# nv-tlabs/LION

Measured on NVIDIA H100. Metric: shapes/sec (1000-step DDPM, 2048 latent pts, B=32), higher is better.
Workload: dtype tf32 (fp32 storage/accumulate)

## Files before the change

### include/lion_b200.h

```cpp
#ifndef LION_B200_H
#define LION_B200_H
#include <stddef.h>
#ifdef __cplusplus
extern "C" {
#endif

typedef struct LionCtx LionCtx;
typedef struct LionModel LionModel;

int lion_version(void);
const char* lion_last_error(void);
int lion_ctx_create(int device, LionCtx** out);
int lion_ctx_destroy(LionCtx* ctx);
int lion_ctx_last_launches(LionCtx* ctx);
int lion_ctx_last_conv_group(LionCtx* ctx);
int lion_ctx_last_conv_stage_taps(LionCtx* ctx);
int lion_ctx_set_conv_whole_slabs(LionCtx* ctx, int on);
int lion_ctx_set_sparse_conv1_dense(LionCtx* ctx, int on);
unsigned lion_ctx_generation(LionCtx* ctx);
int lion_ctx_timeline(LionCtx* ctx, unsigned long long* t_ns, char* names, int max_entries);
size_t lion_ctx_arena_bytes(LionCtx* ctx);
size_t lion_workspace_bytes(LionCtx* ctx);

int lion_avg_voxelize(const float* features, const int* coords, float* out, int* ind, int* cnt,
                      int B, int C, int N, int r, void* stream);
int lion_trilinear_devoxelize(const float* grid, const float* coords, float* out, int* inds, float* wgts,
                              int B, int C, int N, int r, int is_training, void* stream);
int lion_furthest_point_sampling(const float* coords, int* idx, int B, int N, int M, void* stream);
int lion_gather(const float* features, const int* idx, float* out, int B, int C, int N, int M, void* stream);
int lion_ball_query(const float* centers, const float* points, int* out, int B, int N, int M, float radius, int K,
                    void* stream);
int lion_grouping(const float* features, const int* idx, float* out, int B, int C, int N, int M, int U, void* stream);
int lion_three_nn_interpolate(const float* points, const float* centers, const float* centers_features, float* out,
                              int* idx, float* wgt, int B, int C, int N, int M, void* stream);
int lion_voxel_coords(const float* coords, float* norm_coords, int* vox, int B, int N, int r, int normalize, float eps,
                      void* stream);

int lion_avg_voxelize_backward(const float* grad_y , const int* ind , const int* cnt ,
                               float* grad_x , int B, int C, int N, int r, void* stream);
int lion_trilinear_devoxelize_backward(const float* grad_y , const int* inds , const float* wgts ,
                                       float* grad_x , int B, int C, int N, int r, void* stream);
// ... 138 lines not shown
```

### lion_b200/_lib.py

```python
import ctypes as C
import os
import threading

import torch

_HERE = os.path.dirname(os.path.abspath(__file__))
LIB_PATH = os.path.join(_HERE, "csrc", "liblion_b200.so")


class LionError(RuntimeError):
    pass


_lib = None
_lock = threading.Lock()
c_f = C.c_void_p


def _proto(lib):
    i, f, d, sz, vp = C.c_int, C.c_float, C.c_double, C.c_size_t, C.c_void_p
    P = lambda *a: list(a)
    sig = {
        "lion_version": ([], i),
        "lion_last_error": ([], C.c_char_p),
        "lion_ctx_create": (P(i, C.POINTER(vp)), i),
        "lion_ctx_destroy": (P(vp), i),
        "lion_ctx_last_launches": (P(vp), i),
        "lion_ctx_last_conv_group": (P(vp), i),
        "lion_ctx_last_conv_stage_taps": (P(vp), i),
        "lion_ctx_set_conv_whole_slabs": (P(vp, i), i),
        "lion_ctx_set_sparse_conv1_dense": (P(vp, i), i),
        "lion_ctx_arena_bytes": (P(vp), sz),
        "lion_ctx_generation": (P(vp), C.c_uint),
        "lion_ctx_timeline": (P(vp, vp, vp, i), i),
        "lion_avg_voxelize": (P(vp, vp, vp, vp, vp, i, i, i, i, vp), i),
        "lion_trilinear_devoxelize": (P(vp, vp, vp, vp, vp, i, i, i, i, i, vp), i),
        "lion_furthest_point_sampling": (P(vp, vp, i, i, i, vp), i),
        "lion_gather": (P(vp, vp, vp, i, i, i, i, vp), i),
        "lion_ball_query": (P(vp, vp, vp, i, i, i, f, i, vp), i),
        "lion_grouping": (P(vp, vp, vp, i, i, i, i, i, vp), i),
        "lion_three_nn_interpolate": (P(vp, vp, vp, vp, vp, vp, i, i, i, i, vp), i),
        "lion_voxel_coords": (P(vp, vp, vp, i, i, i, i, f, vp), i),
        "lion_avg_voxelize_backward": (P(vp, vp, vp, vp, i, i, i, i, vp), i),
        "lion_trilinear_devoxelize_backward": (P(vp, vp, vp, vp, i, i, i, i, vp), i),
        "lion_grouping_backward": (P(vp, vp, vp, i, i, i, i, i, vp), i),
        "lion_three_nn_interpolate_backward": (P(vp, vp, vp, vp, i, i, i, i, vp), i),
        "lion_gather_backward": (P(vp, vp, vp, i, i, i, i, vp), i),
        "lion_model_create": (P(vp, i, C.POINTER(i), i, C.POINTER(vp), i, C.POINTER(vp)), i),
        "lion_model_destroy": (P(vp), i),
        "lion_model_refresh": (P(vp), i),
        "lion_unet_forward": (P(vp, vp, vp, vp, vp, vp, i, i, vp), i),
        "lion_unet_forward_flags": (P(vp, vp, vp, vp, vp, vp, i, i, i, vp), i),
        "lion_unet_cache_style": (P(vp, vp, vp, i, vp), i),
        "lion_style_encoder_forward": (P(vp, vp, vp, i, i, vp), i),
# ... 232 lines not shown
```

### lion_b200/csrc/common.cuh

```cuda
#pragma once
#include <cuda_runtime.h>
#include <cstdint>
#include <cstdio>
#include <cstdarg>
#include <cstring>
#include <string>
#include <vector>
#include <mutex>

namespace lion {

enum : int { LION_OK = 0, LION_ERR_CUDA = -1, LION_ERR_ARG = -2, LION_ERR_OOM = -3, LION_ERR_STATE = -4 };

void set_error(const char* fmt, ...);
const char* get_error();

#define LION_CHECK_CUDA(expr)                                                          \
  do {                                                                                 \
    cudaError_t _e = (expr);                                                           \
    if (_e != cudaSuccess) {                                                           \
      lion::set_error("%s:%d: %s -> %s", __FILE__, __LINE__, #expr, cudaGetErrorString(_e)); \
      return lion::LION_ERR_CUDA;                                                      \
    }                                                                                  \
  } while (0)
// ... 14 lines not shown

constexpr int LION_MAX_STAMPS = 256;
struct Ctx {
  int device = 0;
  int num_sms = 132;
  int l2_bytes = 50 << 20;
  cudaStream_t stream = nullptr;
  cudaStream_t aux = nullptr;
  char* base = nullptr;
  char* zgrid = nullptr;
  size_t zgrid_cap = 0, zgrid_need = 0;
  size_t cap = 0;
  size_t off = 0;
  size_t peak = 0;
  unsigned generation = 0;
  std::mutex* mu = nullptr;
  bool dry = false;
  int launches = 0;
  int conv_smem_cap = 0;
  int conv_group_blocks = 0;
  int conv_stage_taps = 0;
  bool conv_whole_slabs = false;
  bool sparse_conv1_dense = false;
  unsigned long long* d_stamps = nullptr;
  int n_stamps = 0;
  char stamp_names[LION_MAX_STAMPS][24];

  void reset() { off = 0; peak = 0; launches = 0; zgrid_need = 0; n_stamps = 0; }
  void* alloc(size_t bytes) {
    size_t a = (off + 255) & ~size_t(255);
    off = a + bytes;
    if (off > peak) peak = off;
    if (dry) return (void*)(uintptr_t)(0x1000 + a);
    return base + a;
  }
  template <typename T> T* alloc_n(size_t n) { return (T*)alloc(n * sizeof(T)); }
  size_t mark() const { return off; }
  void release(size_t m) { off = m; }
};

int ctx_reserve(Ctx* c, size_t bytes);

#define LION_LAUNCH_ON(ctx, stream, kernel, grid, block, smem, ...)                    \
  do {                                                                                 \
    if (!(ctx)->dry) {                                                                 \
      kernel<<<(grid), (block), (smem), (stream)>>>(__VA_ARGS__);                      \
// ... 92 lines not shown
```

### lion_b200/csrc/conv_tc.cu

```cuda
#include <algorithm>
#include <type_traits>
#include <cuda_fp16.h>

#include "common.cuh"
#include "model.cuh"
#include "wgmma.cuh"

namespace lion {
namespace tc {

using namespace sm90;

constexpr int CONSUMER_WARPS = 8;
constexpr int THREADS = 32 * CONSUMER_WARPS + 32;
__host__ __device__ constexpr int conv_threads(int BPW) { return BPW == 2 ? 32 * CONSUMER_WARPS + 128 : THREADS; }
constexpr int PRODUCER_REGS = 96, CONSUMER_REGS = 200;
constexpr int MAX_A_STAGES = 16;
constexpr int MAX_B_STAGES = 4;
constexpr int OCC_SMEM = 1024;
__host__ __device__ constexpr int tiles_per_item(int NT) { return NT <= 32 ? 4 : (NT <= 64 ? 2 : 1); }
constexpr int SMEM_BIAS = 128 * 4, SMEM_BARS = 64 * 8 + 128;
__host__ __device__ constexpr int smem_stat(int NT) { return CONSUMER_WARPS * 2 * NT * 4; }
__host__ __device__ constexpr int smem_pool(int NT, int TPG) { return TPG == 1 ? CONSUMER_WARPS * 2 * NT * 4 : 0; }
__host__ __device__ constexpr int smem_fixed(int NT, int TPG) {
// ... 1 lines not shown
}

struct Params {
  const float4* in; const float* w; const float* bias; float4* out; double* ssum; double* ssq;
  int Gin, Gout_store, cout_pad;
  int rows;
  int p_begin, p_end;
  int ntile;
  int ntg, tpg;
  int tg_off[3];
  int tap_off[9];
  int r, rp, nzb, npl, nblk, ib;
  int halo;
  int KG, nchunk;
  int NT;
  int G;
  int B;
  int a_stage_bytes, b_stage_bytes, stage_rows;
  int a_stages;
  int b_stages;
  int tps;
  const unsigned char* occ;
  int occ_stride;
  float* pool_mm;
  int sched;
};

__host__ __device__ __forceinline__ int block_row(int k, int rp, int nzb, int npl) {
  const int x = k / npl, rem = k - x * npl, yb = rem / nzb, zb = rem - yb * nzb;
  return ((x + 1) * rp + 1 + 8 * yb) * rp + 1 + 8 * zb;
}

template <int KG, int TPG, int NT, int NB = 1, typename OP = float>
__device__ __forceinline__ void issue_stage(float (*d)[NT / 2], const uint32_t* a_addr, uint32_t b_addr, uint32_t a_pitch,
                                            uint32_t a_sbo, const int* tap_off) {
  const uint64_t b0 = make_desc(b_addr, NT * 16, 128);
  uint64_t a0[NB];
#pragma unroll
  for (int k = 0; k < NB; ++k) a0[k] = make_desc(a_addr[k], a_pitch, a_sbo);
#pragma unroll
  for (int t = 0; t < TPG; ++t) {
    const uint64_t toff = (uint64_t)(int64_t)(TPG == 1 ? 0 : tap_off[t]);
#pragma unroll
    for (int ks = 0; ks < KG / 2; ++ks)
#pragma unroll
      for (int k = 0; k < NB; ++k) {
// ... 30 lines not shown
    nt = (int)(u / per_nt);
    v0 = u - (long long)nt * per_nt;
    long long run = per_nt - v0;
    if (u_end - u < run) run = u_end - u;
    const long long k2 = (run + G - 1) / G;
    ntile = (int)((run + k2 - 1) / k2);
    u += ntile;
    return true;
  }
};
__device__ __forceinline__ Items make_items(long long U, int ntile_total, int B, int G, int sched) {
  const long long u_begin = U * blockIdx.x / gridDim.x, u_end = U * (blockIdx.x + 1) / gridDim.x;
  Items it{u_begin, u_end, ntile_total, B, G, 0, 0, 0, 0, 0, 0, 0, 0, 0};
  if (sched) {
    const int grid = (int)gridDim.x, q = (int)(U / grid), n_p = (int)(U - (long long)q * grid);
    const int tmax = q + (n_p ? 1 : 0);
    it.mode = 1; it.u = 0; it.u_end = 0;
    it.m = (tmax + G - 1) / G; it.q = q; it.n_p = n_p; it.n_q = grid - n_p;
    it.i = (int)blockIdx.x; it.c_i = (int)(u_begin - (long long)q * blockIdx.x);
    it.big = (int)(u_end - u_begin) > q; it.k = 0;
  }
  return it;
}

__device__ __forceinline__ void halo_mask(int p_lo, int rp, bool& ok_lo, bool& ok_hi) {
  const int p_hi = p_lo + 8;
  const int z0 = p_lo % rp, y0 = (p_lo / rp) % rp, z1 = p_hi % rp, y1 = (p_hi / rp) % rp;
  ok_lo = ok_lo && z0 >= 1 && z0 <= rp - 2 && y0 >= 1 && y0 <= rp - 2;
  ok_hi = ok_hi && z1 >= 1 && z1 <= rp - 2 && y1 >= 1 && y1 <= rp - 2;
}
template <int NT>
__device__ __forceinline__ void stat_add(float* s_stat, int cw, int lane, int col, float x0, float x1, float x2, float x3) {
  const float s0 = red8<0>(x0 + x2), s1 = red8<0>(x1 + x3);
  const float q0 = red8<0>(fmaf(x0, x0, x2 * x2)), q1 = red8<0>(fmaf(x1, x1, x3 * x3));
  if (lane < 4) {
    float* st = s_stat + (cw * 2) * NT + col;
    st[0] += s0; st[1] += s1; st[NT] += q0; st[NT + 1] += q1;
  }
}
template <int NT>
__device__ __forceinline__ void stat_flush(const Params& P, float* s_stat, int et, int b, int n0) {
  asm volatile("bar.sync 1, 256;" ::: "memory");
  if (et < NT) {
    float s = 0.f, qq = 0.f;
#pragma unroll
    for (int w = 0; w < CONSUMER_WARPS; ++w) {
// ... 50 lines not shown
      regs_dec<PRODUCER_REGS>();
      if (warp > CONSUMER_WARPS) return;
    }
    uint32_t sa = 0, pa = 0, sb = 0, pb = 0;
    const uint32_t bytes = (uint32_t)P.stage_rows * 16u;
    const uint32_t sA_addr = smem_u32(sA), sB_addr = smem_u32(sB);
    Items items = items0;
    int nt, ntile;
    long long v0;
    int occ_shape = -1;
    const int slab_floats = P.tpg * KG * NT * 4;
    auto copy_weights = [&](const float* src) {
      mbar_wait<SETREG>(bar_empty_b + 8 * sb, pb ^ 1);
      if (lane == 0) {
        mbar_expect_tx(bar_full_b + 8 * sb, P.b_stage_bytes);
        bulk_g2s(sB_addr + sb * (uint32_t)P.b_stage_bytes, src, P.b_stage_bytes, bar_full_b + 8 * sb);
      }
      if (++sb == B_STAGES) { sb = 0; pb ^= 1; }
    };
    while (items.next(nt, v0, ntile)) {
      const float* wsrc = P.w + (size_t)nt * P.nchunk * P.ntg * slab_floats;
      int my_b = 0, my_t = 0;
      if (lane < ntile) { const int vl = (int)v0 + lane; my_b = vl / ntile_total; my_t = vl - my_b * ntile_total; }
      for (int cc = 0; cc < P.nchunk; ++cc) {
        const int kg_real = min(KG, P.Gin - cc * KG);
        const size_t grp_lane = (size_t)(cc * KG + (lane < kg_real ? lane : 0));
        for (int tg = 0; tg < P.ntg; ++tg) {
          const bool may_skip = P.occ && !(cc == P.nchunk - 1 && tg == P.ntg - 1);
          const float* slab = wsrc + (size_t)(cc * P.ntg + tg) * slab_floats;
          copy_weights(slab);
          for (int j = 0; j < ntile; ++j) {
            const int bj = __shfl_sync(0xffffffffu, my_b, j), tj = __shfl_sync(0xffffffffu, my_t, j);
            long long row0;
            uint32_t cnt = (uint32_t)P.stage_rows;
            if (!BLK) {
              row0 = (long long)P.p_begin + (long long)tj * 128 - P.halo + P.tg_off[tg];
            } else {
              row0 = (long long)block_row(tj * P.ib, P.rp, P.nzb, P.npl) - P.rp - 1 + P.tg_off[tg];
              if (row0 + cnt > (long long)P.rows) cnt = (uint32_t)(P.rows - row0);
            }
            const float4* in_lane = P.in + ((size_t)bj * P.Gin + grp_lane) * P.rows;
            mbar_wait<SETREG>(bar_empty_a + 8 * sa, pa ^ 1);
            bool empty = false;
            if (may_skip) {
              const unsigned char* occ_b = P.occ + (size_t)bj * P.occ_stride;
              if (P.occ_stride <= OCC_SMEM) {
                if (occ_shape != bj) {
                  __syncwarp();
                  for (int k = lane; k < P.occ_stride; k += 32) s_occ[k] = __ldg(occ_b + k);
                  __syncwarp();
                  occ_shape = bj;
                }
                occ_b = s_occ;
              }
// ... 38 lines not shown
      if (s >= 0) { if (lane == 0) mbar_arrive(bar0 + 8 * s); s = -1; }
    };
    while (items.next(nt, v0, ntile)) {
#pragma unroll
      for (int j = 0; j < GT; ++j)
#pragma unroll
        for (int i = 0; i < NACC; ++i) acc[j][i] = 0.0f;
      int g_f = 0, nbw = 0;
      uint32_t boff[GT];
      if (BLK) {
        const int g_b = (int)(v0 / ntile_total);
        g_f = (int)(v0 - (long long)g_b * ntile_total) * P.ib;
        const int nb = min(P.ib, P.nblk - g_f);
        nbw = (nb - wg + 1) / 2;
        const int s_f = block_row(g_f, P.rp, P.nzb, P.npl);
#pragma unroll
        for (int j = 0; j < GT; ++j) {
          const int k = 2 * j + wg < nb ? g_f + 2 * j + wg : g_f;
          boff[j] = (uint32_t)(block_row(k, P.rp, P.nzb, P.npl) - s_f + P.rp + 1) * 16u;
        }
      }
      int pend_a = -1, pend_b = -1;
      bool skip[BLK ? 1 : GT];
      for (int cc = 0; cc < P.nchunk; ++cc) {
        for (int tg = 0; tg < P.ntg; ++tg) {
          const uint32_t sa0 = sa, pa0 = pa;
#pragma unroll
          for (int s = 0; s < NPARTS; ++s) {
            mbar_wait<SETREG>(bar_full_b + 8 * sb, pb);
            const uint32_t b_addr = b_ring + sb * (uint32_t)P.b_stage_bytes;
            const int* toff = P.tap_off + s * TPS;
            bool issued = false;
            sa = sa0; pa = pa0;
#pragma unroll
            for (int j = 0; j < (BLK ? 1 : GT); ++j) {
              if (j < ntile) {
                if (s == 0) {
                  mbar_wait<SETREG>(bar_full_a + 8 * sa, pa);
                  skip[j] = s_skip[sa] != 0;
                  if (skip[j]) { int st = (int)sa; release(st, bar_empty_a); }
                }
                if (!skip[j]) {
                  const uint32_t a_addr = a_ring + sa * (uint32_t)P.a_stage_bytes;
                  wg_fence();
                  if (!BLK) {
                    issue_stage<KG, TPS, NT, 1, OP>(&acc[j], &a_addr, b_addr, a_pitch, a_sbo, toff);
                  } else {
                    uint32_t a_blk[GT];
#pragma unroll
                    for (int k = 0; k < GT; ++k) a_blk[k] = a_addr + boff[k];
                    issue_stage<KG, TPS, NT, GT, OP>(acc, a_blk, b_addr, a_pitch, a_sbo, toff);
                  }
                  wg_commit();
                  wg_wait<1>();
                  release(pend_a, bar_empty_a);
                  release(pend_b, bar_empty_b);
                  if (s == NPARTS - 1) pend_a = (int)sa;
                  issued = true;
                }
                if (++sa == (uint32_t)A_STAGES) { sa = 0; pa ^= 1; }
              }
            }
            if (pend_b >= 0) {
              wg_wait<0>();
              release(pend_a, bar_empty_a);
              release(pend_b, bar_empty_b);
            }
            if (issued) pend_b = (int)sb;
            else { int st = (int)sb; release(st, bar_empty_b); }
            if (++sb == B_STAGES) { sb = 0; pb ^= 1; }
          }
        }
      }
      wg_wait<0>();
      release(pend_a, bar_empty_a);
      release(pend_b, bar_empty_b);
#pragma unroll
      for (int j = 0; j < GT; ++j) fence_regs<NACC>(acc[j]);

      const int n0 = nt * NT;
      asm volatile("bar.sync 1, 256;" ::: "memory");
      if (et < NT) s_bias[et] = P.bias ? P.bias[n0 + et] : 0.0f;
      asm volatile("bar.sync 1, 256;" ::: "memory");
      int b = (int)(v0 / ntile_total);
#pragma unroll
      for (int j = 0; j < GT; ++j) {
        if (j < (BLK ? nbw : ntile)) {
          int tj = 0, p_lo, p_hi;
          bool ok_lo, ok_hi;
          bool in_lo, in_hi;
          if (!BLK) {
            const long long vj = v0 + j;
            const int bj = (int)(vj / ntile_total);
            tj = (int)(vj - (long long)bj * ntile_total);
            if (bj != b) { if (P.ssum) stat_flush<NT>(P, s_stat, et, b, n0); b = bj; }
            p_lo = P.p_begin + tj * 128 + r_lo; p_hi = p_lo + 8;
            in_lo = p_lo < P.p_end; in_hi = p_hi < P.p_end;
            ok_lo = in_lo; ok_hi = in_hi;
            if (TPG != 1) halo_mask(p_lo, P.rp, ok_lo, ok_hi);
          } else {
            const int k = g_f + 2 * j + wg, x = k / P.npl, rem = k - x * P.npl, yb = rem / P.nzb, zb = rem - yb * P.nzb;
            const int y = 1 + 8 * yb + 2 * wq, z = 1 + 8 * zb + (lane >> 2);
            p_lo = ((x + 1) * P.rp + y) * P.rp + z; p_hi = p_lo + P.rp;
            ok_lo = y <= P.r && z <= P.r; ok_hi = y + 1 <= P.r && z <= P.r;
            in_lo = ok_lo; in_hi = ok_hi;
          }
#pragma unroll
          for (int i = 0; i < NT / 8; ++i) {
            const int col = 8 * i + c_lo;
            const float x0 = ok_lo ? acc[j][4 * i + 0] + s_bias[col] : 0.0f, x1 = ok_lo ? acc[j][4 * i + 1] + s_bias[col + 1] : 0.0f;
            const float x2 = ok_hi ? acc[j][4 * i + 2] + s_bias[col] : 0.0f, x3 = ok_hi ? acc[j][4 * i + 3] + s_bias[col + 1] : 0.0f;
            if (P.ssum) stat_add<NT>(s_stat, cw, lane, col, x0, x1, x2, x3);
            if (TPG == 1 && P.pool_mm) {
              const float mn0 = red8<1>(fminf(x0, x2)), mn1 = red8<1>(fminf(x1, x3));
              const float mx0 = red8<2>(fmaxf(x0, x2)), mx1 = red8<2>(fmaxf(x1, x3));
              if (lane < 4) {
                float* sp = s_pool + (cw * 2) * NT + col;
                sp[0] = mn0; sp[1] = mn1; sp[NT] = mx0; sp[NT + 1] = mx1;
              }
            } else {
              const float y0 = __shfl_xor_sync(0xffffffffu, odd ? x0 : x2, 1);
              const float y1 = __shfl_xor_sync(0xffffffffu, odd ? x1 : x3, 1);
              const int g = (n0 + 8 * i + (lane & 2) * 2) >> 2;
              if (g < P.Gout_store) {
                float4* o = P.out + ((size_t)b * P.Gout_store + g) * P.rows;
                if (!odd && in_lo) o[p_lo] = make_float4(x0, x1, y0, y1);
                if (odd && in_hi) o[p_hi] = make_float4(y0, y1, x2, x3);
              }
            }
          }
          if (TPG == 1 && P.pool_mm) {
            const int bar_id = 2 + wg;
            asm volatile("bar.sync %0, 128;" ::"r"(bar_id) : "memory");
            const long long ncent = (long long)P.rows / 32;
            for (int e = et - 128 * wg; e < 2 * NT; e += 128) {
              const int k = e / NT, c = e - k * NT;
              const float* s0 = s_pool + ((4 * wg + 2 * k) * 2) * NT + c;
              const float* s1 = s0 + 2 * NT;
              const float mn = fminf(s0[0], s1[0]), mx = fmaxf(s0[NT], s1[NT]);
              const long long centre = (long long)(P.p_begin + tj * 128 + 64 * wg + 32 * k) >> 5;
              const int ch = n0 + c;
              float* dst = P.pool_mm + ((((size_t)b * (P.cout_pad / 4) + (ch >> 2)) * ncent + centre) * 2) * 4 + (ch & 3);
              dst[0] = mn; dst[4] = mx;
            }
            asm volatile("bar.sync %0, 128;" ::"r"(bar_id) : "memory");
          }
        }
      }
      if (P.ssum) stat_flush<NT>(P, s_stat, et, b, n0);
    }
// ... 113 lines not shown
  });
  return 0;
}

int conv_tc_prepare_f16(Model* m, ConvW& w) {
  if (w.tc16.w || !w.tc.w || w.ntaps != 27 || w.cin_pad != w.cout_pad || w.cout != w.cout_pad) return 0;
  if (!(w.cout_pad == 32 || w.cout_pad == 64 || w.cout_pad == 128)) return 0;
  ConvTcW t = w.tc;
  const int G = w.cin_pad / 8;
  t.KG = conv_tc_kg(w.ntaps, t.NT, G);
  t.nchunk = (G + t.KG - 1) / t.KG;
  if (!((t.NT == 32 && t.KG == 4) || (t.NT == 64 && t.KG == 8) || (t.NT == 128 && t.KG == 4))) return 0;
  const size_t total = (size_t)(w.cout_pad / t.NT) * t.nchunk * t.ntg * t.tpg * t.KG * t.NT * 8;
  __half* w16 = nullptr;
  LION_TRY(m->dmalloc(&w16, total));
  t.w = reinterpret_cast<float*>(w16);
  w.tc16 = t;
  m->repack.push_back([t, w16, wt = w.wt, ntaps = w.ntaps, cin_pad = w.cin_pad, cout_pad = w.cout_pad, total] {
    tc::k_pack_tc16<<<(unsigned)cdivz(total, 256), 256>>>(wt, w16, ntaps, cin_pad, cout_pad, t.NT, t.nchunk, t.ntg, t.tpg, t.KG);
  });
  return 0;
}

bool conv_tc_usable(const ConvW& w, const ConvGeom& geo) {
  if (!w.tc.w) return false;
  if (geo.ntaps != w.ntaps) return false;
  return true;
}

int conv_tc_run(Ctx* c, const ConvW& w, const float4* in, int Gin, float4* out, int Gout_store, double* ssum, double* ssq,
                const ConvGeom& geo, int B, float* pool_mm, bool f16) {
  tc::Params P{};
  if (f16 && !w.tc16.w) { set_error("conv_tc: no FP16 packing of this convolution"); return LION_ERR_STATE; }
  const ConvTcW& T = f16 ? w.tc16 : w.tc;
  if (pool_mm && (w.ntaps != 1 || geo.p_begin != 0 || geo.p_end != geo.rows || geo.rows % 128)) {
    set_error("conv_tc: the pooled epilogue needs a 1x1 convolution over a multiple of 128 rows"); return LION_ERR_ARG;
  }
  P.pool_mm = pool_mm;
  const int NT = T.NT, KG = T.KG, tpg = T.tpg;
  P.in = in; P.w = T.w; P.bias = w.bias; P.out = out; P.ssum = ssum; P.ssq = ssq;
  P.Gin = Gin; P.Gout_store = Gout_store; P.cout_pad = w.cout_pad;
  P.rows = geo.rows; P.p_begin = geo.p_begin; P.p_end = geo.p_end;
  P.ntg = T.ntg; P.tpg = tpg; P.KG = KG; P.nchunk = T.nchunk; P.NT = NT;
  const int slab_bytes = tpg * KG * NT * 16;
  P.B = B;
  P.occ = geo.occ; P.occ_stride = geo.occ_stride;
  const size_t fixed = tc::smem_fixed(NT, tpg);
  const bool blk = w.ntaps == 27 && NT == 128;
  const int ntile_rows = cdiv(geo.p_end - geo.p_begin, 128);
  int ntile;
  P.halo = 0;
  if (w.ntaps == 27) {
    const int rp = geo.rp, r = rp - 2;
    for (int dx = 0; dx < 3; ++dx) P.tg_off[dx] = (dx - 1) * rp * rp;
    for (int dy = 0; dy < 3; ++dy) for (int dz = 0; dz < 3; ++dz) P.tap_off[dy * 3 + dz] = (dy - 1) * rp + (dz - 1);
    P.r = r; P.rp = rp;
  } else {
    P.tg_off[0] = 0; P.tap_off[0] = 0;
  }
  const int n_tiles_n = w.cout_pad / NT;
  if (blk) {
    const int rp = P.rp, r = P.r;
    P.nzb = cdiv(r, 8); P.npl = P.nzb * P.nzb; P.nblk = r * P.npl;
    auto window_rows = [&](int ib) {
      int wrows = 0;
      for (int f = 0; f < P.nblk; f += ib) {
        const int l = std::min(f + ib, P.nblk) - 1;
        wrows = std::max(wrows, tc::block_row(l, rp, P.nzb, P.npl) - tc::block_row(f, rp, P.nzb, P.npl) + 9 * rp + 10);
      }
// ... 25 lines not shown
    }
    int a_stages = (int)((227LL * 1024 - (long long)fixed - b_stages * stage) / P.a_stage_bytes);
    if (c->conv_smem_cap > 0 && a_stages >= 5) {
      const int capped = (int)(((long long)c->conv_smem_cap - (long long)fixed - b_stages * stage) / P.a_stage_bytes);
      if (capped >= 4 && capped < a_stages) a_stages = capped;
    }
    a_stages = std::min(a_stages, tc::MAX_A_STAGES);
    return a_stages >= 2 ? a_stages : 0;
  };
  int b_whole = 0, b_parts = 0;
  const int a_whole = ring(tpg, b_whole);
  const int a_parts = blk && !c->conv_whole_slabs ? ring(3, b_parts) : 0;
  const bool parts = a_parts > a_whole && a_parts >= P.G + 1;
  if (!parts && !a_whole) {
    set_error("conv_tc: shared memory cannot hold the operand pipeline (N=%d, KG=%d)", NT, KG); return LION_ERR_ARG;
  }
  P.tps = parts ? 3 : tpg;
  P.b_stage_bytes = slab_bytes / tpg * P.tps;
  P.b_stages = parts ? b_parts : b_whole;
  const int a_stages = parts ? a_parts : a_whole;
  P.a_stages = a_stages;
  const int b_stages = P.b_stages;
  if (!blk && P.occ && a_stages < 2 * P.G) P.occ = nullptr;
  size_t smem = (size_t)a_stages * P.a_stage_bytes + (size_t)b_stages * P.b_stage_bytes + fixed;
  if (smem > 227 * 1024) { set_error("conv_tc: %zu bytes of shared memory needed", smem); return LION_ERR_ARG; }
  auto grid_for = [&](int nt_per_shape) {
    long long n_units = (long long)nt_per_shape * n_tiles_n * B;
    long long per_cta = (n_units + c->num_sms - 1) / c->num_sms;
    return (int)((n_units + per_cta - 1) / per_cta);
  };
  const int grid = grid_for(ntile);
  tc::Params S = P;
  if (blk && ssum) {
    P.ssum = nullptr; P.ssq = nullptr;
    S.ntile = ntile_rows; S.G = tc::tiles_per_item(NT);
  }
  auto stats = [&]() -> int {
    if (!(blk && ssum)) return 0;
    LION_LAUNCH(c, tc::k_conv_stats<128>, grid_for(ntile_rows), 256, 0, S);
    return check_launch(c, "conv_tc stats");
  };
  const int bpw = blk ? P.ib / 2 : 1;
  c->conv_group_blocks = blk ? P.ib : 0;
  c->conv_stage_taps = P.tps;
#define CONV_TC_CASE_OP(kg, tpg_, nt_, blk_, bpw_, tps_, op)                                              \
  if (f16 == std::is_same<op, __half>::value && KG == kg && tpg == tpg_ && NT == nt_ && blk == blk_ && bpw == bpw_ && P.tps == tps_) { \
// ... 27 lines not shown
```

### lion_b200/csrc/model.cuh

```cuda
#pragma once
#include <functional>
#include <memory>
#include <vector>
#include "common.cuh"

namespace lion {

struct StyleLayer { const float* w; const float* b; int n_out; int out_off; };

struct ConvTcW {
  float* w = nullptr;
  int NT = 0;
  int KG = 0;
  int nchunk = 0;
  int ntg = 0, tpg = 0;
};

struct Cursor {
  const float* const* p;
  int n, i = 0;
  bool bad = false;
  const float* next() {
    if (i >= n) { bad = true; return nullptr; }
    return p[i++];
// ... 131 lines not shown
  }
  ~Model() {
    for (void* q : owned) cudaFree(q);
    for (cudaEvent_t e : events) cudaEventDestroy(e);
    if (aff_cache) cudaFree(aff_cache);
    if (gp) global_prior_free(gp);
  }
};


int make_conv(Model* m, ConvW& w, const float* w_src, const float* b_src, int ntaps, int cin_ref, int cout,
              const std::vector<int>& kmap);
std::vector<int> ident_map(int c);
static inline int roundup(int a, int b) { return (a + b - 1) / b * b; }

struct ConvGeom {
  int ntaps;
  int off[27];
  int rp;
  int rows;
  int p_begin, p_end;
  const unsigned char* occ;
  int occ_stride;
};

int conv_tc_prepare(Model* m, ConvW& w);
int conv_tc_prepare_f16(Model* m, ConvW& w);
bool conv_tc_usable(const ConvW& w, const ConvGeom& geo);
bool ygemm_usable(const ConvW& y);
int ygemm_run(Ctx* c, const ConvW& y, const float4* xc, float* out, int ld, const int* nocc, int B, int N);
bool sa_fused_usable(const SABlk& s);
int sa_fused_run(Ctx* c, const SABlk& s, const float4* feat, const float4* points, const float4* centers, const int* nidx,
                 const float* scale1, const float* shift1, double* ssum, double* ssq, int stat_stride, float* pool_mm,
                 int B, int N);
int conv_tc_run(Ctx* c, const ConvW& w, const float4* in, int Gin, float4* out, int Gout_store, double* ssum,
                double* ssq, const ConvGeom& geo, int B, float* pool_mm = nullptr, bool f16 = false);

}
```

### lion_b200/csrc/net.cu

```cuda
#include <algorithm>
#include <deque>
#include <memory>
#include <cstdlib>
#include <cmath>
#include "common.cuh"
#include "packed_kernels.cuh"
#include "model.cuh"
#include "../../include/lion_b200.h"

namespace lion {

static thread_local char g_err[1024] = "";
void set_error(const char* fmt, ...) {
  va_list ap;
  va_start(ap, fmt);
  vsnprintf(g_err, sizeof(g_err), fmt, ap);
  va_end(ap);
}
const char* get_error() { return g_err; }

int ctx_reserve(Ctx* c, size_t bytes) {
  if (bytes <= c->cap) return 0;
  cudaStreamCaptureStatus st = cudaStreamCaptureStatusNone;
  cudaStreamIsCapturing(c->stream, &st);
// ... 519 lines not shown
      LION_CHECK_CUDA(cudaFuncSetAttribute(k_act_grid<false>, cudaFuncAttributePreferredSharedMemoryCarveout, cudaSharedmemCarveoutMaxShared));
      LION_CHECK_CUDA(cudaFuncSetAttribute(k_act_grid<true>, cudaFuncAttributePreferredSharedMemoryCarveout, cudaSharedmemCarveoutMaxShared));
      LION_CHECK_CUDA(cudaFuncSetAttribute(k_scatter_compact, cudaFuncAttributePreferredSharedMemoryCarveout, cudaSharedmemCarveoutMaxShared));
    }
    const dim3 grid(cdiv(r * r * r, 32 * nwarp), f.B);
    unsigned* mask = f.c->alloc_n<unsigned>((size_t)f.B * cdiv(r * r * r, 32));
    const bool whole = whole_raw || f.c->sparse_conv1_dense;
    if (p.c1.cout_pad == 32)
      LION_LAUNCH(f.c, k_sparse_conv_gather<32>, grid, 32 * nwarp, smem, y, ld, vp->vgrid, p.c1.bias, raw1, s1, q1, p.c1.cout_pad, r, N,
                  mask, whole);
    else
      LION_LAUNCH(f.c, k_sparse_conv_gather<64>, grid, 32 * nwarp, smem, y, ld, vp->vgrid, p.c1.bias, raw1, s1, q1, p.c1.cout_pad, r, N,
                  mask, whole);
    LION_TRY(check_launch(f.c, "sparse conv1"));
    o.ssum = s1; o.ssq = q1;
    o.mask = mask;
  } else {
    LION_TRY(alloc_stats(f, p.c1.cout_pad, &o.ssum, &o.ssq));
    LION_TRY(run_conv(f, p.c1, o.g_in, Gin, raw1, Gout, o.ssum, o.ssq, geo1));
  }
  return 0;
}

static int pvconv_fwd(Fwd& f, const PVConvBlk& p, PF feat, const float4* c4, float4* dst, int Gd, int g_off) {
  int N = feat.R, r = p.r, rp = r + 2, P = rp * rp * rp, Gin = p.cin / 4, Gout = p.cout / 4;
  if (feat.G != Gin) { set_error("PVConv: got %d input channels, expected %d", feat.G * 4, p.cin); return LION_ERR_ARG; }
  VoxPrep* vp;
  LION_TRY(get_vox(f, f.c->stream, c4, N, r, &vp));
  size_t mk = f.c->mark();
  ConvGeom geo = geom_grid(r);
  const ConvW& pw = p.point.conv[0];
  PF rawp;
  AffSrc ap;
  PrepJob jp, j1;
  Conv1Out c1;
  LION_TRY(pvconv_conv1(f, p, feat, vp, 0, f.pv != nullptr, c1, [&]() -> int {
    rawp = alloc_pf(f, Gout, N);
    return conv_gn_deferred(f, pw, feat.p, feat.G, rawp.p, Gout, geom_rows(N), p.point.gn[0], (double)N, ap, jp);
  }));
  const bool sparse1 = c1.sparse;
  float4 *raw1 = c1.raw, *g_in = c1.g_in;
  const unsigned* mask1 = f.c->sparse_conv1_dense ? nullptr : c1.mask;
  AffSrc a1;
  const double V = (double)r * r * r;
  j1 = prep_job(f, p.g1, c1.ssum, c1.ssq, p.c1.cout_pad, V, nullptr, nullptr, a1);
  LION_TRY(run_prep(f, j1, &jp));
  stamp(f.c, f.c->stream, " conv1");
  const bool h2 = f.conv_f16 && p.c2.tc16.w;
  const int Gact = h2 ? Gout / 2 : Gout;
  float4* act1 = alloc_vg(f, Gact, r);
  LION_TRY(poison_vg(f, act1, Gact, r));
  {
    const int nb_act = cdiv(P, 256 * ACT_U);
    const dim3 grid(nb_act + (sparse1 ? 0 : cdiv(N, 256)), Gact, f.B);
    if (h2)
      LION_LAUNCH(f.c, k_act_grid<true>, grid, 256, 0, raw1, act1, a1, Gout, p.cout, rp, P, nb_act, vp->ppos, g_in, Gin, N, mask1,
                  p.c1.bias);
    else
      LION_LAUNCH(f.c, k_act_grid<false>, grid, 256, 0, raw1, act1, a1, Gout, p.cout, rp, P, nb_act, vp->ppos, g_in, Gin, N, mask1,
                  p.c1.bias);
  }
  stamp(f.c, f.c->stream, " act1");
  float4* raw2 = alloc_vg(f, Gout, r);
  LION_TRY(poison_vg(f, raw2, Gout, r));
  AffSrc a2;
  LION_TRY(conv_gn(f, p.c2, act1, Gact, raw2, Gout, geo, p.g2, V, p.se1, p.se2, a2, h2));
  stamp(f.c, f.c->stream, " conv2");
  if (f.pv) {
    PvRecord& R = *f.pv;
    R.raw1 = raw1; R.act1 = act1; R.raw2 = raw2; R.rawp = rawp.p; R.act1_f16 = h2;
    R.a1 = a1; R.ap = ap; R.a2 = a2;
    R.conv2 = !conv_tc_usable(p.c2, geo) ? 0 : f.c->conv_group_blocks ? f.c->conv_group_blocks : 1;
  }
  if (p.has_attn) {
    PF fused = alloc_pf(f, Gout, N);
    LION_LAUNCH(f.c, k_devox_fuse, dim3(cdiv(N, 128), Gout, f.B), 128, 0, raw2, vp->nc, a2.scale, a2.shift, rawp.p, ap,
                fused.p, Gout, p.cout, N, r, P, Gout, 0);
    LION_TRY(check_launch(f.c, "pvconv"));
    if (f.pv) f.pv->fused = fused.p;
    if (Gd != Gout || g_off != 0) {
      PF t = alloc_pf(f, Gout, N);
      LION_TRY(attn_fwd(f, p.attn, fused, t.p, Gout, 0));
      LION_LAUNCH(f.c, k_copy_groups, dim3(cdiv(N, 256), Gout, f.B), 256, 0, t.p, dst, Gout, Gd, g_off, N);
    } else {
      LION_TRY(attn_fwd(f, p.attn, fused, dst, Gd, g_off));
    }
  } else {
    LION_LAUNCH(f.c, k_devox_fuse, dim3(cdiv(N, 128), Gout, f.B), 128, 0, raw2, vp->nc, a2.scale, a2.shift, rawp.p, ap,
                dst, Gout, p.cout, N, r, P, Gd, g_off);
// ... 500 lines not shown
}

}

using namespace lion;

struct LionCtx { Ctx c; std::mutex mu; };
struct LionModel { Model m; };

extern "C" int lion_version(void) { return 100; }
extern "C" const char* lion_last_error(void) { return get_error(); }

extern "C" int lion_ctx_create(int device, LionCtx** out) {
  LION_REQUIRE(out, "lion_ctx_create: null out");
  LION_CHECK_CUDA(cudaSetDevice(device));
  LionCtx* h = new LionCtx();
  h->c.device = device;
  h->c.mu = &h->mu;
  cudaDeviceProp prop;
  LION_CHECK_CUDA(cudaGetDeviceProperties(&prop, device));
  h->c.num_sms = prop.multiProcessorCount;
  h->c.l2_bytes = prop.l2CacheSize;
  LION_CHECK_CUDA(cudaStreamCreateWithFlags(&h->c.aux, cudaStreamNonBlocking));
  { const char* e = getenv("LION_TIMELINE");
    if (e && atoi(e) != 0) LION_CHECK_CUDA(cudaMalloc(&h->c.d_stamps, LION_MAX_STAMPS * sizeof(unsigned long long))); }
  if (prop.major != 9 || prop.minor != 0) {
    set_error("lion_b200 is built for sm_90a only; device %d is sm_%d%d", device, prop.major, prop.minor);
    delete h;
    return LION_ERR_STATE;
  }
  *out = h;
  return 0;
}
extern "C" int lion_ctx_destroy(LionCtx* h) {
  if (!h) return 0;
  if (h->c.base) cudaFree(h->c.base);
  if (h->c.zgrid) cudaFree(h->c.zgrid);
  if (h->c.aux) cudaStreamDestroy(h->c.aux);
  if (h->c.d_stamps) cudaFree(h->c.d_stamps);
  delete h;
  return 0;
}
extern "C" int lion_ctx_last_launches(LionCtx* h) { return h ? h->c.launches : 0; }
extern "C" int lion_ctx_last_conv_group(LionCtx* h) { return h ? h->c.conv_group_blocks : 0; }
extern "C" int lion_ctx_last_conv_stage_taps(LionCtx* h) { return h ? h->c.conv_stage_taps : 0; }
extern "C" int lion_ctx_set_conv_whole_slabs(LionCtx* h, int on) {
  LION_REQUIRE(h, "lion_ctx_set_conv_whole_slabs: null context");
  h->c.conv_whole_slabs = on != 0;
  return 0;
}
extern "C" int lion_ctx_set_sparse_conv1_dense(LionCtx* h, int on) {
  LION_REQUIRE(h, "lion_ctx_set_sparse_conv1_dense: null context");
  h->c.sparse_conv1_dense = on != 0;
  return 0;
}
extern "C" unsigned lion_ctx_generation(LionCtx* h) { return h ? h->c.generation : 0; }
extern "C" int lion_ctx_timeline(LionCtx* h, unsigned long long* t_ns, char* names, int max_entries) {
  LION_REQUIRE(h && t_ns && names && max_entries >= 0, "lion_ctx_timeline: null argument");
  if (!h->c.d_stamps) { set_error("lion_ctx_timeline: the context was created without LION_TIMELINE=1"); return LION_ERR_STATE; }
  int n = h->c.n_stamps < max_entries ? h->c.n_stamps : max_entries;
  LION_CHECK_CUDA(cudaSetDevice(h->c.device));
  LION_CHECK_CUDA(cudaDeviceSynchronize());
  LION_CHECK_CUDA(cudaMemcpy(t_ns, h->c.d_stamps, (size_t)n * sizeof(unsigned long long), cudaMemcpyDeviceToHost));
  for (int i = 0; i < n; ++i) memcpy(names + (size_t)i * 24, h->c.stamp_names[i], 24);
  return n;
}
extern "C" size_t lion_ctx_arena_bytes(LionCtx* h) { return h ? h->c.cap : 0; }
extern "C" size_t lion_workspace_bytes(LionCtx* h) { return h ? h->c.cap + h->c.zgrid_cap : 0; }

extern "C" int lion_model_create(LionCtx* ctx, int kind, const int* desc, int ndesc, const float* const* params,
                                 int nparams, LionModel** out) {
  LION_REQUIRE(ctx && out && (desc || ndesc == 0) && (params || nparams == 0), "lion_model_create: null argument");
  LION_CHECK_CUDA(cudaSetDevice(ctx->c.device));
  std::unique_ptr<LionModel> h(new LionModel());
  Model* m = &h->m;
  m->ctx = &ctx->c; m->kind = kind;
// ... 690 lines not shown
```

### lion_b200/csrc/packed_kernels.cuh

```cuda
#pragma once
#include <cuda_fp16.h>
#include "common.cuh"
#include "point_core.cuh"
#include "model.cuh"

namespace lion {

__device__ __forceinline__ float4 f4_max(float4 a, float4 b) {
  return make_float4(fmaxf(a.x, b.x), fmaxf(a.y, b.y), fmaxf(a.z, b.z), fmaxf(a.w, b.w));
}
__device__ __forceinline__ float4 f4_scale(float4 a, float s) { return make_float4(a.x * s, a.y * s, a.z * s, a.w * s); }
__device__ __forceinline__ float4 f4_add(float4 a, float4 b) { return make_float4(a.x + b.x, a.y + b.y, a.z + b.z, a.w + b.w); }
__device__ __forceinline__ float4 f4_fma(float4 a, float s, float4 c) {
  return make_float4(fmaf(a.x, s, c.x), fmaf(a.y, s, c.y), fmaf(a.z, s, c.z), fmaf(a.w, s, c.w));
}

__global__ void k_make_coords(const float4* __restrict__ x, float4* __restrict__ c4, int total) {
  int i = blockIdx.x * blockDim.x + threadIdx.x;
  if (i >= total) return;
  float4 v = x[i];
  v.w = 0.0f;
  c4[i] = v;
}

// ... 198 lines not shown
#pragma unroll
  for (int k = 0; k < CPL; ++k) { cs[0][k] = cs[1][k] = 0.0f; cq[0][k] = cq[1][k] = 0.0f; }
  const int nlive = max(0, min(32, V - word * 32));
  for (int j = 0; j < nlive; j += 2) {
#pragma unroll
    for (int h = 0; h < 2; ++h) {
      if (j + h < nlive) {
#pragma unroll
        for (int k = 0; k < CPL; ++k) { const float a = acc[(j + h) * PITCH + lane * CPL + k]; cs[h][k] += a; cq[h][k] = fmaf(a, a, cq[h][k]); }
      }
    }
  }
#pragma unroll
  for (int k = 0; k < CPL; ++k) { s_red[0][wid][lane * CPL + k] = cs[0][k] + cs[1][k]; s_red[1][wid][lane * CPL + k] = cq[0][k] + cq[1][k]; }
  __syncthreads();
  if (threadIdx.x < C) {
    float a = 0.0f, qq = 0.0f;
    for (int w = 0; w < nw; ++w) { a += s_red[0][w][threadIdx.x]; qq += s_red[1][w][threadIdx.x]; }
    atomicAdd(ssum + (size_t)b * stat_stride + threadIdx.x, (double)a);
    atomicAdd(ssq + (size_t)b * stat_stride + threadIdx.x, (double)qq);
  }
}

__global__ void k_scatter(const float4* __restrict__ feat, const int* __restrict__ s_order, const int* __restrict__ s_ppos,
                          const int* __restrict__ s_len, float4* __restrict__ grid, int G, int N, int P) {
  int b = blockIdx.z, g = blockIdx.y;
  int s = blockIdx.x * blockDim.x + threadIdx.x;
  if (s >= N) return;
  int pp = s_ppos[(size_t)b * N + s];
  if (pp < 0) return;
  int len = s_len[(size_t)b * N + s];
  float inv = 1.0f / (float)len;
  const float4* f = feat + ((size_t)b * G + g) * N;
  const int* ord = s_order + (size_t)b * N + s;
  float4 acc = f4_scale(f[ord[0]], inv);
  for (int k = 1; k < len; ++k) acc = f4_add(acc, f4_scale(f[ord[k]], inv));
  grid[((size_t)b * G + g) * P + pp] = acc;
}


template <int COT>
__global__ void __launch_bounds__(128)
k_conv_simt(const float4* __restrict__ in, const float* __restrict__ Wt, const float* __restrict__ bias,
            float4* __restrict__ out, double* __restrict__ ssum, double* __restrict__ ssq,
            int Gin, int cin_pad, int cout_pad, int Gout_store, ConvGeom geo) {
  extern __shared__ float s_w[];
// ... 745 lines not shown
```

Measured before the change: 3.214.

## Skip conv2 tiles whose 3x3x3 neighbourhood has no occupied voxels, using class-valued outputs

For the second PVConv convolution, a flag kernel marks 64-voxel blocks whose whole 3x3x3 neighbourhood holds no occupied conv1 voxels. For such blocks the input is just the activated bias, so the output depends only on boundary class. A tiny 5x5x5 class grid is convolved once, and the tensor-core conv skips the MMA for flagged tiles and copies the class values instead. This adds a flag kernel, a small extra conv and branching in the producer/consumer pipeline, which could stall the pipeline when tiles are only partly live.

```diff
diff --git a/include/lion_b200.h b/include/lion_b200.h
--- a/include/lion_b200.h
+++ b/include/lion_b200.h
@@ -17,6 +17,8 @@
 int lion_ctx_last_conv_stage_taps(LionCtx* ctx);
 int lion_ctx_set_conv_whole_slabs(LionCtx* ctx, int on);
 int lion_ctx_set_sparse_conv1_dense(LionCtx* ctx, int on);
+int lion_ctx_set_conv2_class_mode(LionCtx* ctx, int mode);
+int lion_ctx_last_conv2_class_blocks(LionCtx* ctx, long long* flagged, long long* total);
 unsigned lion_ctx_generation(LionCtx* ctx);
 int lion_ctx_timeline(LionCtx* ctx, unsigned long long* t_ns, char* names, int max_entries);
 size_t lion_ctx_arena_bytes(LionCtx* ctx);
diff --git a/lion_b200/_lib.py b/lion_b200/_lib.py
--- a/lion_b200/_lib.py
+++ b/lion_b200/_lib.py
@@ -30,6 +30,8 @@
         "lion_ctx_last_conv_stage_taps": (P(vp), i),
         "lion_ctx_set_conv_whole_slabs": (P(vp, i), i),
         "lion_ctx_set_sparse_conv1_dense": (P(vp, i), i),
+        "lion_ctx_set_conv2_class_mode": (P(vp, i), i),
+        "lion_ctx_last_conv2_class_blocks": (P(vp, vp, vp), i),
         "lion_ctx_arena_bytes": (P(vp), sz),
         "lion_ctx_generation": (P(vp), C.c_uint),
         "lion_ctx_timeline": (P(vp, vp, vp, i), i),
diff --git a/lion_b200/csrc/common.cuh b/lion_b200/csrc/common.cuh
--- a/lion_b200/csrc/common.cuh
+++ b/lion_b200/csrc/common.cuh
@@ -60,6 +60,9 @@
   int conv_stage_taps = 0;
   bool conv_whole_slabs = false;
   bool sparse_conv1_dense = false;
+  int conv2_class_mode = 0;
+  unsigned long long* d_cls_count = nullptr;
+  long long cls_blocks = 0;
   unsigned long long* d_stamps = nullptr;
   int n_stamps = 0;
   char stamp_names[LION_MAX_STAMPS][24];
diff --git a/lion_b200/csrc/conv_tc.cu b/lion_b200/csrc/conv_tc.cu
--- a/lion_b200/csrc/conv_tc.cu
+++ b/lion_b200/csrc/conv_tc.cu
@@ -47,6 +47,10 @@
   int tps;
   const unsigned char* occ;
   int occ_stride;
+  const unsigned char* cls_flag;
+  int cls_stride;
+  const float4* cls;
+  int cls_store;
   float* pool_mm;
   int sched;
 };
@@ -123,6 +127,8 @@
   }
   return it;
 }
+
+__device__ __forceinline__ int cls_of(int v, int r) { return v <= 1 ? 0 : (v >= r ? 2 : 1); }
 
 __device__ __forceinline__ void halo_mask(int p_lo, int rp, bool& ok_lo, bool& ok_hi) {
   const int p_hi = p_lo + 8;
@@ -219,6 +225,12 @@
       const float* wsrc = P.w + (size_t)nt * P.nchunk * P.ntg * slab_floats;
       int my_b = 0, my_t = 0;
       if (lane < ntile) { const int vl = (int)v0 + lane; my_b = vl / ntile_total; my_t = vl - my_b * ntile_total; }
+      unsigned live = (1u << ntile) - 1u;
+      if (!BLK && P.cls_flag) {
+        const unsigned char* fl = P.cls_flag + (size_t)my_b * P.cls_stride + 2 * my_t;
+        live = __ballot_sync(0xffffffffu, lane < ntile && !(__ldg(fl) && __ldg(fl + 1)));
+      }
+      if (!live) continue;
       for (int cc = 0; cc < P.nchunk; ++cc) {
         const int kg_real = min(KG, P.Gin - cc * KG);
         const size_t grp_lane = (size_t)(cc * KG + (lane < kg_real ? lane : 0));
@@ -227,6 +239,7 @@
           const float* slab = wsrc + (size_t)(cc * P.ntg + tg) * slab_floats;
           copy_weights(slab);
           for (int j = 0; j < ntile; ++j) {
+            if (!((live >> j) & 1u)) continue;
             const int bj = __shfl_sync(0xffffffffu, my_b, j), tj = __shfl_sync(0xffffffffu, my_t, j);
             long long row0;
             uint32_t cnt = (uint32_t)P.stage_rows;
@@ -311,7 +324,22 @@
       }
       int pend_a = -1, pend_b = -1;
       bool skip[BLK ? 1 : GT];
-      for (int cc = 0; cc < P.nchunk; ++cc) {
+      unsigned live = (1u << ntile) - 1u, mine = ~0u;
+      if (!BLK && P.cls_flag) {
+        live = 0u; mine = 0u;
+#pragma unroll
+        for (int j = 0; j < GT; ++j) {
+          if (j < ntile) {
+            const long long vj = v0 + j;
+            const int bj = (int)(vj / ntile_total), tj = (int)(vj - (long long)bj * ntile_total);
+            const unsigned char* fl = P.cls_flag + (size_t)bj * P.cls_stride + 2 * tj;
+            const bool f0 = __ldg(fl) != 0, f1 = __ldg(fl + 1) != 0;
+            if (!(f0 && f1)) live |= 1u << j;
+            if (!(wg ? f1 : f0)) mine |= 1u << j;
+          }
+        }
+      }
+      for (int cc = 0; cc < (live ? P.nchunk : 0); ++cc) {
         for (int tg = 0; tg < P.ntg; ++tg) {
           const uint32_t sa0 = sa, pa0 = pa;
 #pragma unroll
@@ -323,10 +351,10 @@
             sa = sa0; pa = pa0;
 #pragma unroll
             for (int j = 0; j < (BLK ? 1 : GT); ++j) {
-              if (j < ntile) {
+              if ((live >> j) & 1u) {
                 if (s == 0) {
                   mbar_wait<SETREG>(bar_full_a + 8 * sa, pa);
-                  skip[j] = s_skip[sa] != 0;
+                  skip[j] = s_skip[sa] != 0 || !((mine >> j) & 1u);
                   if (skip[j]) { int st = (int)sa; release(st, bar_empty_a); }
                 }
                 if (!skip[j]) {
@@ -357,6 +385,11 @@
             }
             if (issued) pend_b = (int)sb;
             else { int st = (int)sb; release(st, bar_empty_b); }
+            if ((live & ~mine) && pend_b >= 0) {
+              wg_wait<0>();
+              release(pend_a, bar_empty_a);
+              release(pend_b, bar_empty_b);
+            }
             if (++sb == B_STAGES) { sb = 0; pb ^= 1; }
           }
         }
@@ -387,6 +420,20 @@
             in_lo = p_lo < P.p_end; in_hi = p_hi < P.p_end;
             ok_lo = in_lo; ok_hi = in_hi;
             if (TPG != 1) halo_mask(p_lo, P.rp, ok_lo, ok_hi);
+            if (!((mine >> j) & 1u)) {
+              const float4* cb = P.cls + (size_t)b * (P.cout_pad / 4) * 125 + n0 / 4;
+#pragma unroll
+              for (int h = 0; h < 2; ++h) {
+                const int p = h ? p_hi : p_lo, x = p / (P.rp * P.rp), y = (p / P.rp) % P.rp, z = p % P.rp;
+                const int row = ((cls_of(x, P.r) + 1) * 5 + cls_of(y, P.r) + 1) * 5 + cls_of(z, P.r) + 1;
+                const float* src = reinterpret_cast<const float*>(cb + ((lane & 3) >> 1) * 125 + row) + 2 * (lane & 1);
+#pragma unroll
+                for (int i = 0; i < NT / 8; ++i) {
+                  const float2 v = __ldg(reinterpret_cast<const float2*>(src + (size_t)2 * 125 * 4 * i));
+                  acc[j][4 * i + 2 * h] = v.x; acc[j][4 * i + 2 * h + 1] = v.y;
+                }
+              }
+            }
           } else {
             const int k = g_f + 2 * j + wg, x = k / P.npl, rem = k - x * P.npl, yb = rem / P.nzb, zb = rem - yb * P.nzb;
             const int y = 1 + 8 * yb + 2 * wq, z = 1 + 8 * zb + (lane >> 2);
@@ -394,11 +441,13 @@
             ok_lo = y <= P.r && z <= P.r; ok_hi = y + 1 <= P.r && z <= P.r;
             in_lo = ok_lo; in_hi = ok_hi;
           }
+          const bool cmp = (mine >> j) & 1u, st = cmp || P.cls_store;
 #pragma unroll
           for (int i = 0; i < NT / 8; ++i) {
             const int col = 8 * i + c_lo;
-            const float x0 = ok_lo ? acc[j][4 * i + 0] + s_bias[col] : 0.0f, x1 = ok_lo ? acc[j][4 * i + 1] + s_bias[col + 1] : 0.0f;
-            const float x2 = ok_hi ? acc[j][4 * i + 2] + s_bias[col] : 0.0f, x3 = ok_hi ? acc[j][4 * i + 3] + s_bias[col + 1] : 0.0f;
+            float x0 = acc[j][4 * i + 0], x1 = acc[j][4 * i + 1], x2 = acc[j][4 * i + 2], x3 = acc[j][4 * i + 3];
+            if (cmp) { x0 += s_bias[col]; x1 += s_bias[col + 1]; x2 += s_bias[col]; x3 += s_bias[col + 1]; }
+            x0 = ok_lo ? x0 : 0.0f; x1 = ok_lo ? x1 : 0.0f; x2 = ok_hi ? x2 : 0.0f; x3 = ok_hi ? x3 : 0.0f;
             if (P.ssum) stat_add<NT>(s_stat, cw, lane, col, x0, x1, x2, x3);
             if (TPG == 1 && P.pool_mm) {
               const float mn0 = red8<1>(fminf(x0, x2)), mn1 = red8<1>(fminf(x1, x3));
@@ -413,8 +462,8 @@
               const int g = (n0 + 8 * i + (lane & 2) * 2) >> 2;
               if (g < P.Gout_store) {
                 float4* o = P.out + ((size_t)b * P.Gout_store + g) * P.rows;
-                if (!odd && in_lo) o[p_lo] = make_float4(x0, x1, y0, y1);
-                if (odd && in_hi) o[p_hi] = make_float4(y0, y1, x2, x3);
+                if (!odd && in_lo && st) o[p_lo] = make_float4(x0, x1, y0, y1);
+                if (odd && in_hi && st) o[p_hi] = make_float4(y0, y1, x2, x3);
               }
             }
           }
@@ -574,6 +623,8 @@
   return 0;
 }
 
+bool conv_tc_row_tiles_3x3(const ConvW& w) { return w.tc.w && w.ntaps == 27 && w.tc.NT <= 64; }
+
 bool conv_tc_usable(const ConvW& w, const ConvGeom& geo) {
   if (!w.tc.w) return false;
   if (geo.ntaps != w.ntaps) return false;
@@ -597,6 +648,7 @@
   const int slab_bytes = tpg * KG * NT * 16;
   P.B = B;
   P.occ = geo.occ; P.occ_stride = geo.occ_stride;
+  P.cls_flag = geo.cls_flag; P.cls_stride = geo.cls_stride; P.cls = geo.cls; P.cls_store = geo.cls_store ? 1 : 0;
   const size_t fixed = tc::smem_fixed(NT, tpg);
   const bool blk = w.ntaps == 27 && NT == 128;
   const int ntile_rows = cdiv(geo.p_end - geo.p_begin, 128);
@@ -668,6 +720,10 @@
   P.a_stages = a_stages;
   const int b_stages = P.b_stages;
   if (!blk && P.occ && a_stages < 2 * P.G) P.occ = nullptr;
+  if (P.cls_flag && (blk || w.ntaps != 27 || P.occ || 2 * ntile > P.cls_stride)) {
+    set_error("conv_tc: class-valued blocks are for 3x3x3 row tiles of a dense input"); return LION_ERR_ARG;
+  }
+  if (a_stages < P.G) P.cls_flag = nullptr;
   size_t smem = (size_t)a_stages * P.a_stage_bytes + (size_t)b_stages * P.b_stage_bytes + fixed;
   if (smem > 227 * 1024) { set_error("conv_tc: %zu bytes of shared memory needed", smem); return LION_ERR_ARG; }
   auto grid_for = [&](int nt_per_shape) {
diff --git a/lion_b200/csrc/model.cuh b/lion_b200/csrc/model.cuh
--- a/lion_b200/csrc/model.cuh
+++ b/lion_b200/csrc/model.cuh
@@ -177,11 +177,16 @@
   int p_begin, p_end;
   const unsigned char* occ;
   int occ_stride;
+  const unsigned char* cls_flag;
+  int cls_stride;
+  const float4* cls;
+  bool cls_store;
 };
 
 int conv_tc_prepare(Model* m, ConvW& w);
 int conv_tc_prepare_f16(Model* m, ConvW& w);
 bool conv_tc_usable(const ConvW& w, const ConvGeom& geo);
+bool conv_tc_row_tiles_3x3(const ConvW& w);
 bool ygemm_usable(const ConvW& y);
 int ygemm_run(Ctx* c, const ConvW& y, const float4* xc, float* out, int ld, const int* nocc, int B, int N);
 bool sa_fused_usable(const SABlk& s);
diff --git a/lion_b200/csrc/net.cu b/lion_b200/csrc/net.cu
--- a/lion_b200/csrc/net.cu
+++ b/lion_b200/csrc/net.cu
@@ -565,6 +565,31 @@
   return 0;
 }
 
+static int conv2_classes(Fwd& f, const PVConvBlk& p, const VoxPrep* vp, const unsigned* mask1, const float4* raw1,
+                         const AffSrc& a1, bool h2, ConvGeom& geo) {
+  const int r = p.r, rp = r + 2, Gout = p.cout / 4, Gc = p.c2.cout_pad / 4, Gact = h2 ? Gout / 2 : Gout;
+  const int nblk = 2 * cdiv(r * rp * rp, 128);
+  if (nblk > vp->occ_stride) { set_error("conv2 classes: %d blocks exceed the flag stride %d", nblk, vp->occ_stride); return LION_ERR_STATE; }
+  unsigned char* flags = f.c->alloc_n<unsigned char>((size_t)f.B * vp->occ_stride);
+  unsigned* zmask = f.c->alloc_n<unsigned>((size_t)f.B);
+  LION_TRY(memset_async(f.c, f.c->d_cls_count, 0, sizeof(unsigned long long)));
+  LION_LAUNCH(f.c, k_conv2_flags, dim3(cdiv(nblk, 8), f.B), 256, 0, mask1, r, nblk, flags, vp->occ_stride, zmask, f.c->d_cls_count);
+  f.c->cls_blocks = (long long)f.B * nblk;
+  const int CP = 125, guard = 64;
+  float4* cg = f.c->alloc_n<float4>((size_t)f.B * Gact * CP + 2 * guard) + guard;
+  if (h2)
+    LION_LAUNCH(f.c, k_act_grid<true>, dim3(1, Gact, f.B), 256, 0, raw1, cg, a1, Gout, p.cout, 5, CP, 1, nullptr, nullptr, 0, 0,
+                zmask, p.c1.bias);
+  else
+    LION_LAUNCH(f.c, k_act_grid<false>, dim3(1, Gact, f.B), 256, 0, raw1, cg, a1, Gout, p.cout, 5, CP, 1, nullptr, nullptr, 0, 0,
+                zmask, p.c1.bias);
+  LION_TRY(check_launch(f.c, "conv2 classes"));
+  float4* cls = f.c->alloc_n<float4>((size_t)f.B * Gc * CP);
+  LION_TRY(run_conv(f, p.c2, cg, Gact, cls, Gc, nullptr, nullptr, geom_grid(3), nullptr, h2));
+  geo.cls_flag = flags; geo.cls_stride = vp->occ_stride; geo.cls = cls; geo.cls_store = f.pv != nullptr;
+  return 0;
+}
+
 static int pvconv_fwd(Fwd& f, const PVConvBlk& p, PF feat, const float4* c4, float4* dst, int Gd, int g_off) {
   int N = feat.R, r = p.r, rp = r + 2, P = rp * rp * rp, Gin = p.cin / 4, Gout = p.cout / 4;
   if (feat.G != Gin) { set_error("PVConv: got %d input channels, expected %d", feat.G * 4, p.cin); return LION_ERR_ARG; }
@@ -606,8 +631,14 @@
   stamp(f.c, f.c->stream, " act1");
   float4* raw2 = alloc_vg(f, Gout, r);
   LION_TRY(poison_vg(f, raw2, Gout, r));
+  ConvGeom geo2 = geo;
+  if (mask1 && r >= 3 && f.c->conv2_class_mode != 1 && conv_tc_row_tiles_3x3(p.c2)) {
+    if (f.c->conv2_class_mode == 2 && !f.pv)
+      LION_TRY(memset_async(f.c, raw2, 0xff, sizeof(float4) * f.B * Gout * (size_t)P));
+    LION_TRY(conv2_classes(f, p, vp, mask1, raw1, a1, h2, geo2));
+  }
   AffSrc a2;
-  LION_TRY(conv_gn(f, p.c2, act1, Gact, raw2, Gout, geo, p.g2, V, p.se1, p.se2, a2, h2));
+  LION_TRY(conv_gn(f, p.c2, act1, Gact, raw2, Gout, geo2, p.g2, V, p.se1, p.se2, a2, h2));
   stamp(f.c, f.c->stream, " conv2");
   if (f.pv) {
     PvRecord& R = *f.pv;
@@ -1154,6 +1185,8 @@
   h->c.num_sms = prop.multiProcessorCount;
   h->c.l2_bytes = prop.l2CacheSize;
   LION_CHECK_CUDA(cudaStreamCreateWithFlags(&h->c.aux, cudaStreamNonBlocking));
+  LION_CHECK_CUDA(cudaMalloc(&h->c.d_cls_count, sizeof(unsigned long long)));
+  LION_CHECK_CUDA(cudaMemset(h->c.d_cls_count, 0, sizeof(unsigned long long)));
   { const char* e = getenv("LION_TIMELINE");
     if (e && atoi(e) != 0) LION_CHECK_CUDA(cudaMalloc(&h->c.d_stamps, LION_MAX_STAMPS * sizeof(unsigned long long))); }
   if (prop.major != 9 || prop.minor != 0) {
@@ -1170,6 +1203,7 @@
   if (h->c.zgrid) cudaFree(h->c.zgrid);
   if (h->c.aux) cudaStreamDestroy(h->c.aux);
   if (h->c.d_stamps) cudaFree(h->c.d_stamps);
+  if (h->c.d_cls_count) cudaFree(h->c.d_cls_count);
   delete h;
   return 0;
 }
@@ -1184,6 +1218,20 @@
 extern "C" int lion_ctx_set_sparse_conv1_dense(LionCtx* h, int on) {
   LION_REQUIRE(h, "lion_ctx_set_sparse_conv1_dense: null context");
   h->c.sparse_conv1_dense = on != 0;
+  return 0;
+}
+extern "C" int lion_ctx_set_conv2_class_mode(LionCtx* h, int mode) {
+  LION_REQUIRE(h && mode >= 0 && mode <= 2, "lion_ctx_set_conv2_class_mode: null context or mode not 0-2");
+  h->c.conv2_class_mode = mode;
+  return 0;
+}
+extern "C" int lion_ctx_last_conv2_class_blocks(LionCtx* h, long long* flagged, long long* total) {
+  LION_REQUIRE(h && flagged && total, "lion_ctx_last_conv2_class_blocks: null argument");
+  unsigned long long n = 0;
+  LION_CHECK_CUDA(cudaSetDevice(h->c.device));
+  LION_CHECK_CUDA(cudaDeviceSynchronize());
+  LION_CHECK_CUDA(cudaMemcpy(&n, h->c.d_cls_count, sizeof(n), cudaMemcpyDeviceToHost));
+  *flagged = (long long)n; *total = h->c.cls_blocks;
   return 0;
 }
 extern "C" unsigned lion_ctx_generation(LionCtx* h) { return h ? h->c.generation : 0; }
diff --git a/lion_b200/csrc/packed_kernels.cuh b/lion_b200/csrc/packed_kernels.cuh
--- a/lion_b200/csrc/packed_kernels.cuh
+++ b/lion_b200/csrc/packed_kernels.cuh
@@ -244,6 +244,41 @@
   }
 }
 
+__global__ void __launch_bounds__(256) k_conv2_flags(const unsigned* __restrict__ mask, int r, int nblk,
+                                                     unsigned char* __restrict__ flags, int stride,
+                                                     unsigned* __restrict__ zmask, unsigned long long* __restrict__ count) {
+  __shared__ int s_n;
+  const int b = blockIdx.y, lane = threadIdx.x & 31, k = blockIdx.x * 8 + (threadIdx.x >> 5);
+  const int rp = r + 2, p_end = (rp - 1) * rp * rp;
+  const unsigned* mb = mask + (size_t)b * ((r * r * r + 31) / 32);
+  if (threadIdx.x == 0) s_n = 0;
+  if (blockIdx.x == 0 && threadIdx.x == 0) zmask[b] = 0u;
+  __syncthreads();
+  bool hit = false;
+  if (k < nblk) {
+    for (int h = 0; h < 2; ++h) {
+      const int p = rp * rp + 64 * k + 32 * h + lane;
+      const int x = p / (rp * rp), y = (p / rp) % rp, z = p % rp;
+      if (p >= p_end || y < 1 || y > r || z < 1 || z > r) continue;
+      for (int dx = -1; dx <= 1; ++dx)
+        for (int dy = -1; dy <= 1; ++dy)
+          for (int dz = -1; dz <= 1; ++dz) {
+            const int xx = x + dx, yy = y + dy, zz = z + dz;
+            if (xx < 1 || xx > r || yy < 1 || yy > r || zz < 1 || zz > r) continue;
+            const int q = ((xx - 1) * r + (yy - 1)) * r + (zz - 1);
+            hit |= ((__ldg(mb + (q >> 5)) >> (q & 31)) & 1u) != 0;
+          }
+    }
+  }
+  const bool flag = !__any_sync(0xffffffffu, hit);
+  if (k < nblk && lane == 0) {
+    flags[(size_t)b * stride + k] = flag ? 1 : 0;
+    if (flag) atomicAdd(&s_n, 1);
+  }
+  __syncthreads();
+  if (threadIdx.x == 0 && s_n) atomicAdd(count, (unsigned long long)s_n);
+}
+
 __global__ void k_scatter(const float4* __restrict__ feat, const int* __restrict__ s_order, const int* __restrict__ s_ppos,
                           const int* __restrict__ s_len, float4* __restrict__ grid, int G, int N, int P) {
   int b = blockIdx.z, g = blockIdx.y;
```

Result: faster. 3.326, median of 6 (+3.5%).
